# winstonww/ReacherDistilation

Measured on AMD Instinct MI355X. Metric: Reacher env-steps/sec (rollout+distill step) at 1/2/4/8 MI355X; student MSE, higher is better.
Workload: dtype f32; 1 GPU; c4; description=BASELINE config 4: 262,144 envs per GPU, RCCL student-grad all-reduce, MSE, fp32, envs_per_gpu=262144, envs_total=262144, student=MlpPolicy 2x64 tanh (5060 params, f32), teacher=MlpPolicy 2x64 tanh, loss=mse, act_with=teacher, optimizer=TF1 Adam lr 0.0001, 1 step per env-step, parallelism=dp1, collective=none, f32_mode=split

## Files before the change

include/reacher_distill.h:

```cpp
#ifndef REACHER_DISTILL_H
#define REACHER_DISTILL_H
#include <stdint.h>

#include "reacher.h"
#include "reacher_comm.h"

#ifdef __cplusplus
extern "C" {
#endif

#define RDD_LOSS_MSE 0
#define RDD_LOSS_KL 1
#define RDD_ACT_TEACHER 0
#define RDD_ACT_STUDENT 1

typedef struct {
    int64_t n_envs;
    int64_t n_envs_global;
    int64_t env_base;
    uint64_t seed;
    int32_t loss;
    int32_t act_with;
    float lr, beta1, beta2, eps;
    int32_t grid;
    int32_t metrics_len;
    int32_t stagger;
    int32_t student_dtype;
    int32_t accum_steps;
    int32_t f32_split;
    int32_t group_envs;
} rdd_config;

#define RDD_DTYPE_F32 0
#define RDD_DTYPE_BF16 1


#define RDD_STAGGER_GROUP 32

typedef struct rdd_trainer rdd_trainer;

int rdd_create(rdd_trainer** out, const rdd_config* cfg, int device, void* hip_stream);
int rdd_destroy(rdd_trainer* tr);
int rdd_param_count(void);
int rdd_set_stream(rdd_trainer* tr, void* hip_stream);

int rdd_set_teacher(rdd_trainer* tr, const float* params, const float* ob_mean, const float* ob_std);
int rdd_set_student(rdd_trainer* tr, const float* params, const float* ob_mean, const float* ob_std);
int rdd_get_student(rdd_trainer* tr, float* params);

int rdd_reset(rdd_trainer* tr);

int rdd_rollout(rdd_trainer* tr);
int rdd_apply(rdd_trainer* tr);
int rdd_step(rdd_trainer* tr);
int rdd_rollout_accum(rdd_trainer* tr);
int rdd_step_accum(rdd_trainer* tr);
int rdd_rollout_obs(rdd_trainer* tr, const float* obs, int64_t n, int64_t n_global);
int rdd_step_obs(rdd_trainer* tr, const float* obs, int64_t n);
int rdd_rollout_rows(rdd_trainer* tr, const float* obs, const float* t_pdflat, int64_t n, int64_t n_global);
int rdd_step_rows(rdd_trainer* tr, const float* obs, const float* t_pdflat, int64_t n);

#define RDD_STAGE_ROLLOUT 1
#define RDD_STAGE_REDUCE 2
#define RDD_STAGE_APPLY 3
#define RDD_STAGE_REDUCE_APPLY 4
#define RDD_STAGE_REDUCE_ACCUM 5
#define RDD_STAGE_REDUCE_ACCUM_APPLY 6
int rdd_launch_stage(rdd_trainer* tr, int stage);
float* rdd_grad_buffer(rdd_trainer* tr);
int rdd_bind_grad_buffer(rdd_trainer* tr, float* grad);
int rdd_bind_comm(rdd_trainer* tr, rd_comm* comm);
int rdd_allreduce_grad(rdd_trainer* tr);

int rdd_forward(rdd_trainer* tr, const float* obs, int64_t n, float* t_pdflat, float* s_pdflat);

#define RDD_EVAL_TEACHER 0
#define RDD_EVAL_STUDENT 1
typedef struct {
    int64_t n_envs;
    int64_t env_base;
    uint64_t seed;
    int32_t policy;
    int32_t episodes;
    int32_t first_episode;
    int32_t grid;
    const float* draws;
} rdd_eval_config;
int rdd_evaluate(rdd_trainer* tr, const rdd_eval_config* cfg, float* returns, float* final_dist, float* records);

int rdd_get_env_state(rdd_trainer* tr, float* state);
int rdd_set_env_state(rdd_trainer* tr, const float* state);

int rdd_get_counter(rdd_trainer* tr, int64_t* steps);
int rdd_get_counters(rdd_trainer* tr, int64_t* env_steps, int64_t* opt_steps);
int rdd_read_metrics(rdd_trainer* tr, int64_t count, double* out);
int rdd_last_layout(const rdd_trainer* tr, int32_t out[4]);

#ifdef __cplusplus
}
#endif
#endif
```

reacherdistilation_amd/csrc/distill.hip:

```cpp
#include <hip/hip_runtime.h>
#include <stdint.h>

#include <new>

#include "../../include/reacher_distill.h"
#include "rd_comm_impl.h"
#include "rd_common.h"
#include "rd_host.h"
#include "rd_device.h"
#include "rd_physics.h"

namespace {

using rd::f32x4, rd::mfma, rd::ld4, rd::st4, rd::wave_sum, rd::wave_sync, rd::kTanhScale, rd::tanh_pre, rd::load_state;

#ifdef RD_STAMPS
#define STAMP(idx)                                                                      \
    do {                                                                                \
        __builtin_amdgcn_sched_barrier(0);                                              \
        unsigned long long t_;                                                          \
        asm volatile("s_memtime %0\n\ts_waitcnt lgkmcnt(0)" : "=s"(t_)::"memory");     \
        __builtin_amdgcn_sched_barrier(0);                                              \
        if (lane == 0 && a.dbg) a.dbg[(blockIdx.x * WAVES + wave) * NSTAMP + (idx)] += t_;   \
    } while (0)
#define RTSTAMP(idx)                                                                    \
    do {                                                                                \
        __builtin_amdgcn_sched_barrier(0);                                              \
        const unsigned long long t_ = __builtin_amdgcn_s_memrealtime();                 \
        __builtin_amdgcn_sched_barrier(0);                                              \
        if (lane == 0 && a.dbg) a.dbg[(blockIdx.x * WAVES + wave) * NSTAMP + (idx)] += t_;   \
    } while (0)
#else
#define STAMP(idx) do {} while (0)
#define RTSTAMP(idx) do {} while (0)
#endif

#include "distill_layout.h"
#include "distill_forward.h"
#include "distill_reduce.h"
#include "distill_rollout.h"
#include "distill_eval.h"

}

struct rdd_trainer {
    rdd_config cfg{};
    int device = 0;
    hipStream_t stream = nullptr;
    int grid = 0;
    rd::DeviceAllocs mem;
    float* state = nullptr;
    float* tnet = nullptr;
    float* snet = nullptr;
    float* timg = nullptr;
    float* simg = nullptr;
    float* m = nullptr;
    float* v = nullptr;
    float* grad = nullptr;
    float* own_grad = nullptr;
    float* ws = nullptr;
    float* hist = nullptr;
    uint32_t* ctl = nullptr;
    unsigned long long* dbg = nullptr;
    int last_grid = 0;
    int last_gs = GROUP, last_hlp = 0, last_mode = 0;
    int ws_rows = 0;
    int cus = 0;
    int gs = GROUP;
    int accum = 1;
    rd_comm* comm = nullptr;
};

namespace {

int group_envs(int64_t n, int pairs_total, int fixed) {
    if (fixed) return fixed;
    if (n >= (int64_t)GROUP * pairs_total) return 64;
    if (n >= (int64_t)32 * pairs_total) return 32;
    return 16;
}

int teacher_kind(const rdd_trainer* t) { return t->cfg.f32_split ? IMG_SPLIT : IMG_F32; }
int student_kind(const rdd_trainer* t) {
    return t->cfg.student_dtype == RDD_DTYPE_BF16 ? IMG_BF16 : (t->cfg.f32_split ? IMG_SPLIT : IMG_F32);
}
int image_floats(int kind, bool student) {
    if (kind == IMG_SPLIT) return student ? NETX_S : NETX;
    if (kind == IMG_BF16) return NETB_S;
    return student ? NET_S : NET;
}

int grid_for(int64_t n, int gs, int cap) {
    const int64_t want = ((n + gs - 1) / gs + PAIRS - 1) / PAIRS;
    return (int)(want < cap ? want : cap);
}

ReduceArgs reduce_args(const rdd_trainer* t, int reduce, int adam, int accum) {
    ReduceArgs a;
    a.ws = t->ws;
    a.nblk = t->last_grid;
    a.grad = t->grad;
    a.params = t->snet;
    a.m = t->m;
    a.v = t->v;
    a.ctl = t->ctl;
    a.hist = t->hist;
    a.hist_len = t->cfg.metrics_len;
    a.reduce = reduce;
    a.adam = adam;
    a.accum = accum;
    a.bump_env = reduce;
    a.bump_opt = adam;
    a.lr = t->cfg.lr;
    a.b1 = t->cfg.beta1;
    a.b2 = t->cfg.beta2;
    a.eps = t->cfg.eps;
    a.simg = t->simg;
    a.img_kind = student_kind(t);
    a.xerr = rd_comm_device_err(t->comm);
    return a;
}

int launch_rollout(rdd_trainer* t, const float* obs_in = nullptr, int64_t n_obs = 0, int64_t n_obs_global = 0,
                   const float* tflat_in = nullptr, int ksteps = 1) {
    RolloutArgs a;
    a.ksteps = ksteps;
    a.n = obs_in ? n_obs : t->cfg.n_envs;
    a.obs_in = obs_in;
    a.timg = t->timg;
    a.simg = t->simg;
    a.env_base = t->cfg.env_base;
    a.seed = t->cfg.seed;
    a.state = t->state;
    a.tnet = tflat_in ? tflat_in : t->tnet;
    a.snet = t->snet;
    a.ctl = t->ctl;
    a.ws = t->ws;
    a.loss = t->cfg.loss;
    a.act_student = t->cfg.act_with == RDD_ACT_STUDENT;
    a.stagger = t->cfg.stagger;
    a.dbg = t->dbg;
    a.inv_n_global = obs_in ? 1.0f / (float)n_obs_global : 1.0f / ((float)t->cfg.n_envs_global * (float)t->accum);
    int grid = t->grid;
    a.gs = t->gs;
    if (obs_in) {
        a.gs = group_envs(n_obs, t->ws_rows * PAIRS, t->cfg.group_envs);
        grid = grid_for(n_obs, a.gs, t->ws_rows);
    }
    const bool bs = t->cfg.student_dtype == RDD_DTYPE_BF16, spl = t->cfg.f32_split != 0;
    const int64_t ngroups = (a.n + a.gs - 1) / a.gs;
    const bool hlp = !bs && !tflat_in && a.gs == TILE && ngroups <= 2 * (int64_t)t->ws_rows &&
                     t->cfg.group_envs == 0 &&
                     ksteps == 1;
    if (hlp) grid = (int)((ngroups + 1) / 2);
    t->last_grid = grid;
    t->last_gs = a.gs;
    t->last_hlp = hlp;
    t->last_mode = tflat_in ? 2 : (obs_in ? 1 : 0);
    void (*k)(RolloutArgs) =
        bs ? (spl ? rollout_kernel<true, true, true, MD_TEACHER, false, true>
                  : rollout_kernel<true, false, true, MD_TEACHER>)
           : hlp ? (spl ? rollout_kernel<false, true, false, MD_HELPER> : rollout_kernel<false, false, false, MD_HELPER>)
                 : (spl ? rollout_kernel<false, true, false, MD_TEACHER> : rollout_kernel<false, false, false, MD_TEACHER>);
    if (ksteps > 1)
        k = bs ? (spl ? rollout_kernel<true, true, false, MD_TEACHER, true> : rollout_kernel<true, false, false, MD_TEACHER, true>)
               : (spl ? rollout_kernel<false, true, false, MD_TEACHER, true> : rollout_kernel<false, false, false, MD_TEACHER, true>);
    if (tflat_in)
        k = bs ? rollout_kernel<true, false, false, MD_ROWS>
               : (spl ? rollout_kernel<false, true, false, MD_ROWS> : rollout_kernel<false, false, false, MD_ROWS>);
    hipLaunchKernelGGL(k, dim3(grid), dim3(BLOCK), 0, t->stream, a);
    RD_HIP(hipGetLastError(), "rollout_kernel launch");
    return RD_OK;
}

int launch_reduce(rdd_trainer* t, int reduce, int adam, int accum = 0) {
    const ReduceArgs a = reduce_args(t, reduce, adam, accum);
    hipLaunchKernelGGL(reduce_adam_kernel, dim3(RED_GRID), dim3(RED_BLOCK), 0, t->stream, a);
    RD_HIP(hipGetLastError(), "reduce_adam_kernel launch");
    return RD_OK;
}

}

extern "C" {

int rdd_param_count(void) { return P_TOT; }

int rdd_set_stream(rdd_trainer* t, void* hip_stream) {
    if (!t) return rd::set_error(RD_EINVAL, "rdd_set_stream: null handle");
    t->stream = (hipStream_t)hip_stream;
    return RD_OK;
}

int rdd_create(rdd_trainer** out, const rdd_config* cfg, int device, void* hip_stream) {
    if (!out || !cfg) return rd::set_error(RD_EINVAL, "rdd_create: null argument");
    if (cfg->n_envs <= 0 || cfg->n_envs_global < cfg->n_envs || cfg->env_base < 0 ||
        cfg->n_envs > ((int64_t)1 << 31) || (cfg->loss != RDD_LOSS_MSE && cfg->loss != RDD_LOSS_KL) ||
        (cfg->act_with != RDD_ACT_TEACHER && cfg->act_with != RDD_ACT_STUDENT) || !(cfg->lr > 0) ||
        cfg->grid < 0 || cfg->metrics_len < 0 || (cfg->stagger != 0 && cfg->stagger != 1) ||
        (cfg->student_dtype != RDD_DTYPE_F32 && cfg->student_dtype != RDD_DTYPE_BF16) || cfg->accum_steps < 0 ||
        (cfg->f32_split != 0 && cfg->f32_split != 1) ||
        (cfg->group_envs != 0 && cfg->group_envs != 16 && cfg->group_envs != 32 && cfg->group_envs != 64))
        return rd::set_error(RD_EINVAL, "rdd_create: bad config");
    rd::DeviceGuard g(device);
    RD_HIP(g.err, "rdd_create: hipSetDevice");
    rdd_trainer* t = new (std::nothrow) rdd_trainer();
    if (!t) return rd::set_error(RD_EINVAL, "rdd_create: out of host memory");
    t->cfg = *cfg;
    if (t->cfg.metrics_len == 0) t->cfg.metrics_len = 4096;
    t->accum = cfg->accum_steps > 1 ? cfg->accum_steps : 1;
    t->device = device;
    t->stream = (hipStream_t)hip_stream;
    t->cus = rd::cu_count(device);
    const int cap = cfg->grid > 0 ? cfg->grid : t->cus;
    t->ws_rows = cap;
    t->gs = group_envs(cfg->n_envs, cap * PAIRS, cfg->group_envs);
    t->grid = grid_for(cfg->n_envs, t->gs, cap);
    t->last_grid = t->grid;
    t->last_gs = t->gs;
    const size_t netf = P_TOT + 2 * OBD;
    rd::DeviceAllocs& mem = t->mem;
    mem.stream = t->stream;
    mem.zeroed(&t->state, (size_t)8 * cfg->n_envs);
    mem.zeroed(&t->tnet, netf);
    mem.zeroed(&t->snet, netf);
    mem.zeroed(&t->timg, image_floats(teacher_kind(t), false));
    mem.zeroed(&t->simg, image_floats(student_kind(t), true));
    mem.zeroed(&t->m, P_TOT);
    mem.zeroed(&t->v, P_TOT);
    mem.zeroed(&t->own_grad, P_TOT);
    t->grad = t->own_grad;
    mem.zeroed(&t->ws, (size_t)t->ws_rows * P_WS);
    mem.zeroed(&t->hist, (size_t)t->cfg.metrics_len * N_MET);
    mem.zeroed(&t->ctl, 16);
#ifdef RD_STAMPS
    mem.zeroed(&t->dbg, (size_t)t->ws_rows * WAVES * NSTAMP);
#endif
    if (mem.err != hipSuccess) {
        const hipError_t e = mem.err;
        rdd_destroy(t);
        return rd::hip_fail(e, "rdd_create: allocation");
    }
    *out = t;
    return RD_OK;
}

int rdd_destroy(rdd_trainer* t) {
    if (!t) return RD_OK;
    rd::DeviceGuard g(t->device);
    t->mem.free_all();
    delete t;
    return RD_OK;
}

static int set_net(rdd_trainer* t, float* dst, const float* params, const float* mu, const float* sd,
                   const char* what) {
    if (!t || !params || !mu || !sd) return rd::set_error(RD_EINVAL, "%s: null argument", what);
    rd::DeviceGuard g(t->device);
    RD_HIP(g.err, what);
    if (int rc = rd::upload_net(what, dst, params, P_TOT, mu, sd, OBD, t->stream)) return rc;
    const bool student = dst == t->snet;
    const int kind = student ? student_kind(t) : teacher_kind(t);
    hipLaunchKernelGGL(pack_net_kernel, dim3(1), dim3(256), 0, t->stream, dst, student ? t->simg : t->timg,
                       image_floats(kind, student), student ? 1 : 0, kind);
    RD_HIP(hipGetLastError(), what);
    return RD_OK;
}

int rdd_set_teacher(rdd_trainer* t, const float* p, const float* mu, const float* sd) {
    return set_net(t, t ? t->tnet : nullptr, p, mu, sd, "rdd_set_teacher");
}

// ... 223 lines not shown
    RD_HIP(g.err, "rdd_set_env_state");
    const int64_t n = t->cfg.n_envs;
    uint32_t bad = 0;
    RD_HIP(hipMemsetAsync(t->ctl + 14, 0, sizeof(uint32_t), t->stream), "rdd_set_env_state");
    hipLaunchKernelGGL(check_state_kernel, dim3((unsigned)((n + 255) / 256)), dim3(256), 0, t->stream, n, state,
                       t->ctl + 14);
    RD_HIP(hipGetLastError(), "rdd_set_env_state: check_state_kernel launch");
    RD_HIP(hipMemcpyAsync(&bad, t->ctl + 14, sizeof(bad), hipMemcpyDeviceToHost, t->stream), "rdd_set_env_state");
    RD_HIP(hipStreamSynchronize(t->stream), "rdd_set_env_state");
    if (bad)
        return rd::set_error(RD_EINVAL,
                             "rdd_set_env_state: a joint angle outside the fused rollout's range (|q0| < %g, |q1| <= %g "
                             "rad, finite); the gym-API env (rd_set_state) takes any state",
                             (double)rd::kRolloutMaxQ0, (double)rd::kRolloutMaxQ1);
    RD_HIP(hipMemcpyAsync(t->state, state, sizeof(float) * 8 * n, hipMemcpyDeviceToDevice, t->stream),
           "rdd_set_env_state");
    return RD_OK;
}

static int read_ctl(rdd_trainer* t, uint32_t (&c)[16], const char* what) {
    rd::DeviceGuard g(t->device);
    RD_HIP(g.err, what);
    RD_HIP(hipMemcpyAsync(c, t->ctl, sizeof(c), hipMemcpyDeviceToHost, t->stream), what);
    RD_HIP(hipStreamSynchronize(t->stream), what);
    if (c[8]) return rd::set_error(RD_EINVAL, "%s: a rollout's producer/consumer hand-off timed out", what);
    if (c[13]) return rd::set_error(RD_ECOMM, "%s: a gradient exchange failed; its optimiser step was skipped", what);
    return RD_OK;
}

int rdd_get_counter(rdd_trainer* t, int64_t* steps) {
    if (!t || !steps) return rd::set_error(RD_EINVAL, "rdd_get_counter: null argument");
    uint32_t c[16];
    if (int rc = read_ctl(t, c, "rdd_get_counter")) return rc;
    *steps = c[0];
    return RD_OK;
}

int rdd_get_counters(rdd_trainer* t, int64_t* env_steps, int64_t* opt_steps) {
    if (!t) return rd::set_error(RD_EINVAL, "rdd_get_counters: null handle");
    uint32_t c[16];
    if (int rc = read_ctl(t, c, "rdd_get_counters")) return rc;
    if (env_steps) *env_steps = c[0];
    if (opt_steps) *opt_steps = c[1];
    return RD_OK;
}

int rdd_read_metrics(rdd_trainer* t, int64_t count, double* out) {
    if (!t || !out || count < 0) return rd::set_error(RD_EINVAL, "rdd_read_metrics: bad argument");
    int64_t steps = 0;
    if (int rc = rdd_get_counters(t, nullptr, &steps)) return rc;
    return rd::read_ring("rdd_read_metrics", "steps", t->hist, t->cfg.metrics_len, N_MET, steps, count, out);
}

int rdd_last_layout(const rdd_trainer* t, int32_t out[4]) {
    if (!t || !out) return rd::set_error(RD_EINVAL, "rdd_last_layout: null argument");
    out[0] = t->last_gs;
    out[1] = t->last_grid;
    out[2] = t->last_hlp;
    out[3] = t->last_mode;
    return RD_OK;
}

#ifdef RD_STAMPS
int rdd_debug_stamps(rdd_trainer* t, unsigned long long* out, int64_t cap) {
    if (!t || !out || !t->dbg) return rd::set_error(RD_EINVAL, "rdd_debug_stamps: bad argument");
    const int64_t cnt = (int64_t)t->ws_rows * WAVES * NSTAMP;
    if (cap < cnt) return rd::set_error(RD_EINVAL, "rdd_debug_stamps: need %lld", (long long)cnt);
    RD_HIP(hipStreamSynchronize(t->stream), "rdd_debug_stamps");
    RD_HIP(hipMemcpy(out, t->dbg, sizeof(unsigned long long) * cnt, hipMemcpyDeviceToHost), "rdd_debug_stamps");
    RD_HIP(hipMemset(t->dbg, 0, sizeof(unsigned long long) * cnt), "rdd_debug_stamps");
    return (int)cnt;
}
#endif

}
```

reacherdistilation_amd/csrc/distill_rollout.h:

```cpp
#pragma once

struct RolloutArgs {
    int64_t n, env_base;
    uint64_t seed;
    float* state;
    const float* tnet;
    const float* snet;
    uint32_t* ctl;
    float* ws;
    int loss, act_student, stagger;
    float inv_n_global;
    int gs;
    int ksteps;
    unsigned long long* dbg;
    const float* obs_in;
    const float* timg;
    const float* simg;
};

__device__ __forceinline__ bool wait_ge(const uint32_t* f, uint32_t target, uint32_t* err) {
    for (uint32_t spins = 0;; ++spins) {
        if (__hip_atomic_load(f, __ATOMIC_ACQUIRE, __HIP_MEMORY_SCOPE_WORKGROUP) >= target) return true;
        if (spins > SPIN_LIMIT) {
            if ((threadIdx.x & 63) == 0) __hip_atomic_store(err, 1u, __ATOMIC_RELAXED, __HIP_MEMORY_SCOPE_AGENT);
            return false;
        }
        __builtin_amdgcn_s_sleep(1);
    }
}

__device__ __forceinline__ void publish(uint32_t* f, uint32_t v) {
    __hip_atomic_store(f, v, __ATOMIC_RELEASE, __HIP_MEMORY_SCOPE_WORKGROUP);
}

__device__ __forceinline__ float env_step_group(const RolloutArgs& a, uint32_t C, int64_t i, bool valid, float act0,
                                                float act1, rd::State& st, float& met_n) {
    const uint32_t iu = (uint32_t)i;
    const float rew = rd::env_step<false>(st, act0, act1);
    const int64_t gid = a.env_base + i;
    const uint32_t u = C + (a.stagger ? (uint32_t)((gid / RDD_STAGGER_GROUP) % rd::kEpisodeSteps) : 0u);
    const bool done_step = (u % rd::kEpisodeSteps) == rd::kEpisodeSteps - 1;
    if (done_step) {
        float dr[6];
        rd::philox_draw(a.seed, (uint64_t)gid, u / rd::kEpisodeSteps + 1, dr);
        rd::env_reset(st, dr);
    }
    if (!valid) return 0.0f;
    rd::store_state(a.state, a.n, iu, st, done_step);
    met_n += 1.0f;
    return rew;
}

constexpr int MD_TEACHER = 0, MD_ROWS = 1, MD_HELPER = 2;
template <bool BS, bool SPL, bool CP, int MD, bool KS = false, bool TC = false>
__global__ __launch_bounds__(BLOCK, 2) void rollout_kernel(RolloutArgs a) {
    constexpr bool TGT = MD == MD_ROWS, HLP = MD == MD_HELPER;
    static_assert(!TC || (BS && MD == MD_TEACHER && !KS), "teacher on the consumer: bf16 student, K = 1");
    constexpr int P_TM = CP ? P_ACT : P_SACT;
    static_assert(!HLP || !BS, "helper pairs: f32 student kernels only");
    constexpr int TN = TGT ? 0 : img_t(SPL), SN = img_s(BS, SPL);
    __shared__ __attribute__((aligned(16))) float lds[TN + SN + PAIRS * PSCR];
    float* LT = lds;
    float* LS = lds + TN;
    const int wave = threadIdx.x >> 6, lane = threadIdx.x & 63;
    const int j = lane & 15, g = lane >> 4;
    const int pair = wave & (PAIRS - 1);
    const bool producer = wave < PAIRS;
    uint32_t* flags = reinterpret_cast<uint32_t*>(lds + TN + SN + pair * PSCR + P_FLAGS);
    uint32_t* err = a.ctl + 8;

    RTSTAMP(16);
    STAMP(0);
    const int gs = a.gs;
    const uint32_t n32 = (uint32_t)a.n;
    const uint32_t ngroups = (n32 + (uint32_t)gs - 1) / (uint32_t)gs;
    static_assert(!KS || (!CP && MD == MD_TEACHER), "K-step launches: teacher mode, producer-side env step");
    if constexpr (KS) {
        if (a.obs_in) {
            if (threadIdx.x == 0) __hip_atomic_store(a.ctl + 8, 1u, __ATOMIC_RELAXED, __HIP_MEMORY_SCOPE_AGENT);
            return;
        }
    }
    if constexpr (HLP) {
        if (ngroups > 2u * gridDim.x) {
            if (threadIdx.x == 0) __hip_atomic_store(a.ctl + 8, 1u, __ATOMIC_RELAXED, __HIP_MEMORY_SCOPE_AGENT);
            return;
        }
    }
    const bool helper = HLP && pair >= 2;
    const uint32_t gstride = gridDim.x * (HLP ? 2 : PAIRS);
    const uint32_t gfirst = helper ? ngroups : blockIdx.x * (HLP ? 2 : PAIRS) + pair;
    rd::State st0{};
    if (producer && !a.obs_in && gfirst < ngroups && lane < gs && gfirst * gs + lane < a.n)
        load_state(a.state, a.n, (uint32_t)(gfirst * gs + lane), st0);
    const uint32_t og = blockIdx.x * 2 + (pair & 1);
    const bool hstep = helper && producer && !a.obs_in && !a.act_student;
    if constexpr (HLP) {
        if (hstep && og < ngroups && lane < gs && og * gs + lane < a.n)
            load_state(a.state, a.n, (uint32_t)(og * gs + lane), st0);
    }
    static_assert(NET % 4 == 0 && NET_S % 4 == 0, "16-B images");
    float* PS = lds + TN + SN + pair * PSCR;
    const bool first_obs = producer && gfirst < ngroups;
    auto group_obs = [&](uint32_t k, uint32_t i, bool lvalid, rd::State& st) {
        float ob[OBD];
        if (a.obs_in) {
#pragma unroll
            for (int q = 0; q < OBD; ++q) ob[q] = lvalid ? a.obs_in[(size_t)i * OBD + q] : 0.0f;
        } else {
            rd::observe<false>(st, ob);
// ... 64 lines not shown
            STAMP(8);
            const uint32_t Ck = C + kk;
            const uint32_t base = grp * (uint32_t)gs;
            const uint32_t i = base + (uint32_t)lane;
            const bool lvalid = lane < gs && i < n32;
            float* obs = PS + P_SO;
            float* act = PS + P_ACT;
            rd::State st{};
            if (k == 0) {
                st = st0;
            } else if (resident) {
                if (lvalid) st = st0;
                group_obs(k, i, lvalid, st);
            } else {
                if (!a.obs_in && lvalid) load_state(a.state, a.n, i, st);
                group_obs(k, i, lvalid, st);
            }
            STAMP(11);
            wave_sync();
            if constexpr (TC) publish(flags + 2, k + 1);
            const int ntile = (int)min((uint32_t)(gs / TILE), (n32 - base + TILE - 1) / TILE);
            for (int t = 0; t < ntile; ++t) {
                const bool tvalid = base + TILE * t + j < a.n;
                const float* obt = obs + TILE * t * SOS;
                f32x4 H1[4], H2[4];
                float mt0, mt1, ms0, ms1;
                float rl0 = tl0, rl1 = tl1, rr0 = rtv0, rr1 = rtv1;
                STAMP(10);
                if constexpr (TGT) {
                    const uint32_t row = base + TILE * t + j;
                    const f32x4 tq = tvalid ? ld4(a.tnet + (size_t)row * 4) : f32x4{0.f, 0.f, 0.f, 0.f};
                    if constexpr (BS) mlp_forward_bf16(LS, obt, j, g, H1, H2, ms0, ms1);
                    else if constexpr (SPL) mlp_forward_split_t<true>(LS, obt, j, g, H1, H2, ms0, ms1);
                    else mlp_forward(LS, obt, j, g, H1, H2, ms0, ms1);
                    mt0 = tq[0];
                    mt1 = tq[1];
                    rl0 = tq[2];
                    rl1 = tq[3];
                    rr0 = 1.0f / __expf(2.0f * rl0);
                    rr1 = 1.0f / __expf(2.0f * rl1);
                } else if constexpr (HLP) {
                    if (k == 0) {
                        if constexpr (SPL) mlp_forward_split_t<true>(LS, obt, j, g, H1, H2, ms0, ms1);
                        else mlp_forward<true>(LS, obt, j, g, H1, H2, ms0, ms1);
                        const float* hp = lds + TN + SN + (pair + 2) * PSCR;
                        if (!(ok = wait_ge(reinterpret_cast<const uint32_t*>(hp + P_FLAGS), 1u, err))) break;
                        mt0 = hp[P_ACT + 2 * j];
                        mt1 = hp[P_ACT + 2 * j + 1];
                    } else {
                        if constexpr (SPL) mlp_forward_pair_split(LT, LS, obt, j, g, H1, H2, mt0, mt1, ms0, ms1);
                        else mlp_forward_pair<true>(LT, LS, obt, j, g, H1, H2, mt0, mt1, ms0, ms1);
                    }
                } else if constexpr (BS) {
                    if (TC && (t & 1)) {
                        mlp_forward_bf16(LS, obt, j, g, H1, H2, ms0, ms1);
                        if (!(ok = wait_ge(flags + 3, ++tct, err))) break;
                        mt0 = PS[P_TM + 2 * j];
                        mt1 = PS[P_TM + 2 * j + 1];
                    } else {
                    if constexpr (SPL) mlp_forward_split(LT, obt, j, g, mt0, mt1);
                    else mlp_forward<CP || KS || TC>(LT, obt, j, g, H1, H2, mt0, mt1);
                    mlp_forward_bf16(LS, obt, j, g, H1, H2, ms0, ms1);
                    }
                } else {
                    if constexpr (SPL) mlp_forward_pair_split(LT, LS, obt, j, g, H1, H2, mt0, mt1, ms0, ms1);
                    else mlp_forward_pair<false, kPairFence>(LT, LS, obt, j, g, H1, H2, mt0, mt1, ms0, ms1);
                }
                STAMP(12);
                const float d0 = ms0 - mt0, d1 = ms1 - mt1;
                float dm0, dm1, dl0 = 0.0f, dl1 = 0.0f, lossv;
                if (a.loss == RDD_LOSS_MSE) {
                    dm0 = d0 * a.inv_n_global;
                    dm1 = d1 * a.inv_n_global;
                    lossv = (d0 * d0 + d1 * d1) * (0.5f * a.inv_n_global);
                } else {
                    dm0 = d0 * rr0;
                    dm1 = d1 * rr1;
                    dl0 = sv0 * rr0 - 1.0f;
                    dl1 = sv1 * rr1 - 1.0f;
                    lossv = (rl0 - sl0 + (sv0 + d0 * d0) * (0.5f * rr0) - 0.5f) +
                            (rl1 - sl1 + (sv1 + d1 * d1) * (0.5f * rr1) - 0.5f);
                }
                if (!tvalid) { dm0 = dm1 = dl0 = dl1 = 0.0f; }
                if (g == 0 && tvalid) {
                    met_l += lossv;
                    met_m += d0 * d0 + d1 * d1;
                    gb3a += dm0; gb3b += dm1; gls0 += dl0; gls1 += dl1;
                    if (!CP) {
                        act[(TILE * t + j) * 2] = a.act_student ? ms0 : mt0;
                        act[(TILE * t + j) * 2 + 1] = a.act_student ? ms1 : mt1;
                    }
                }
                f32x4 dZ[4];
#pragma unroll
                for (int fb = 0; fb < 4; ++fb) {
                    const f32x4 wa = ld4(LS + SW3 + (16 * fb + 4 * g) * 2);
                    const f32x4 wb = ld4(LS + SW3 + (16 * fb + 4 * g) * 2 + 4);
                    const float w0[4] = {wa[0], wa[2], wb[0], wb[2]}, w1[4] = {wa[1], wa[3], wb[1], wb[3]};
#pragma unroll
                    for (int r = 0; r < 4; ++r) {
                        const float h = H2[fb][r];
                        gw3a[fb][r] = fmaf(h, dm0, gw3a[fb][r]);
                        gw3b[fb][r] = fmaf(h, dm1, gw3b[fb][r]);
                        dZ[fb][r] = fmaf(w0[r], dm0, w1[r] * dm1) * fmaf(-h, h, 1.0f);
                    }
                }
                STAMP(2);
                if (!(ok = wait_ge(flags + 1, tiles, err))) break;
                STAMP(3);
                float* h1t = PS + P_H1T;
                float* dzt = PS + P_DZT;
#pragma unroll
                for (int fb = 0; fb < 4; ++fb) {
                    st4(h1t + j * SAS + 16 * fb + 4 * g, H1[fb]);
                    st4(dzt + j * SAS + 16 * fb + 4 * g, dZ[fb]);
                }
                if (lane < TILE * SOS / 4) st4(PS + P_SOB + 4 * lane, ld4(obt + 4 * lane));
                if (CP && g == 0) {
                    PS[P_SACT + 2 * j] = a.act_student ? ms0 : mt0;
// ... 269 lines not shown
                const float* OP = lds + TN + SN + (pair & 1) * PSCR;
                STAMP(20);
                ok = wait_ge(reinterpret_cast<const uint32_t*>(OP + P_FLAGS), 1u, err);
                STAMP(21);
                if (ok) {
                    const float* h1t = OP + P_H1T;
                    const float* dzt = OP + P_DZT;
                    if constexpr (SPL) {
                        float x32[2][8], y32[2][8];
#pragma unroll
                        for (int e = 0; e < 8; ++e)
#pragma unroll
                            for (int b = 0; b < 2; ++b) {
                                x32[b][e] = h1t[(8 * h32 + e) * SAS + 32 * b + c32];
                                y32[b][e] = dzt[(8 * h32 + e) * SAS + 32 * b + c32];
                            }
#pragma unroll
                        for (int b = 0; b < 2; ++b)
                            gb2s[b] += ((y32[b][0] + y32[b][1]) + (y32[b][2] + y32[b][3])) +
                                       ((y32[b][4] + y32[b][5]) + (y32[b][6] + y32[b][7]));
                        dw2_split32(x32, y32, gW2s);
                    } else {
                    float x[4][4], y[4][4];
#pragma unroll
                    for (int s = 0; s < 4; ++s)
#pragma unroll
                        for (int b = 0; b < 4; ++b) {
                            x[s][b] = h1t[(4 * s + g) * SAS + 16 * b + j];
                            y[s][b] = dzt[(4 * s + g) * SAS + 16 * b + j];
                        }
#pragma unroll
                        for (int s = 0; s < 4; ++s) {
#pragma unroll
                            for (int b = 0; b < 4; ++b) gb2[b] += y[s][b];
#pragma unroll
                            for (int mb = 0; mb < 4; ++mb) {
                                fence_begin<true>(gW2[mb]);
#pragma unroll
                                for (int nb = 0; nb < 4; ++nb) gW2[mb][nb] = mfma(x[s][mb], y[s][nb], gW2[mb][nb]);
                                fence_end<true>(gW2[mb]);
                            }
                        }
                    }
                }
                STAMP(22);
            }
        }
        uint32_t gi = 0, tcc = 0;
        for (uint32_t kk = 0;; ++kk) {
        for (uint32_t grp = gfirst; ok && grp < ngroups; grp += gstride, ++gi) {
            const uint32_t base = grp * (uint32_t)gs;
            const int ntile = (int)min((uint32_t)(gs / TILE), (n32 - base + TILE - 1) / TILE);
            if constexpr (TC) {
                if (!(ok = wait_ge(flags + 2, gi + 1, err))) break;
            }
            for (int t = 0; ok && t < ntile; ++t) {
                if constexpr (TC) {
                    if (!(t & 1) && t + 1 < ntile) {
                        const float* obt = PS + P_SO + TILE * (t + 1) * SOS;
                        float m0, m1;
                        if constexpr (SPL) {
                            mlp_forward_split(LT, obt, j, g, m0, m1);
                        } else {
                            f32x4 h1[4], h2[4];
                            mlp_forward<true>(LT, obt, j, g, h1, h2, m0, m1);
                        }
                        if (g == 0) {
                            PS[P_TM + 2 * j] = m0;
                            PS[P_TM + 2 * j + 1] = m1;
                        }
                        publish(flags + 3, ++tcc);
                    }
                }
                ok = bwd_tile(t);
            }
            if (!ok) break;
            end_group(base, C + kk);
        }
        if (!KS || !ok || kk + 1 >= (uint32_t)a.ksteps) break;
        }
#pragma unroll
        for (int x = 0; x < 4; ++x) gb2[x] = xsum32(xsum16(gb2[x]));
#pragma unroll
        for (int x = 0; x < 2; ++x) gb2s[x] = xsum32(gb2s[x]);
        if constexpr (CP) { met_r = wave_sum(met_r); met_n = wave_sum(met_n); }
        STAMP(6);
        __syncthreads();
        STAMP(9);
        float* R = lds + pair * RPAD;
        if constexpr (D32) {
#pragma unroll
            for (int mb = 0; mb < 2; ++mb)
#pragma unroll
                for (int nb = 0; nb < 2; ++nb)
#pragma unroll
                    for (int r = 0; r < 16; ++r)
                        R[(12 + 32 * mb + (r & 3) + 8 * (r >> 2) + 4 * h32) * RROW + 32 * nb + c32] = gW2s[mb][nb][r];
        } else {
#pragma unroll
        for (int mb = 0; mb < 4; ++mb)
#pragma unroll
            for (int nb = 0; nb < 4; ++nb)
#pragma unroll
                for (int r = 0; r < 4; ++r) R[(12 + 16 * mb + 4 * g + r) * RROW + 16 * nb + j] = gW2[mb][nb][r];
        }
        if (g < 3) {
#pragma unroll
            for (int nb = 0; nb < 4; ++nb)
#pragma unroll
                for (int r = 0; r < 4; ++r) R[(4 * g + r) * RROW + 16 * nb + j] = gW1[nb][r];
        }
        if constexpr (D32) {
            if (h32 == 0) {
#pragma unroll
                for (int nb = 0; nb < 2; ++nb) R[RSHIFT + P_B2 + 32 * nb + c32] = gb2s[nb];
            }
        } else if (g == 0) {
#pragma unroll
// ... 23 lines not shown
```

reacherdistilation_amd/distill.py:

```python
from __future__ import annotations

import ctypes
from dataclasses import dataclass

import numpy as np
import torch

from . import _native as nat
from .dist import allreduce_sum_, replicas_identical, shard
from .policy import P_TOT, MlpPolicyParams, student_init, synthetic_teacher

P = nat.P
I32, I64, U64, F32, INT = nat.I32, nat.I64, nat.U64, nat.F32, nat.INT

LOSSES = {"mse": 0, "kl": 1}
ACTORS = {"teacher": 0, "student": 1}
DTYPES = {"f32": 0, "bf16": 1}


class RddConfig(ctypes.Structure):
    _fields_ = [("n_envs", I64), ("n_envs_global", I64), ("env_base", I64), ("seed", U64),
                ("loss", I32), ("act_with", I32), ("lr", F32), ("beta1", F32), ("beta2", F32),
                ("eps", F32), ("grid", I32), ("metrics_len", I32), ("stagger", I32),
                ("student_dtype", I32), ("accum_steps", I32), ("f32_split", I32), ("group_envs", I32)]


class RddEvalConfig(ctypes.Structure):
    _fields_ = [("n_envs", I64), ("env_base", I64), ("seed", U64), ("policy", I32), ("episodes", I32),
                ("first_episode", I32), ("grid", I32), ("draws", P)]


@dataclass
class EvalResult:
    returns: torch.Tensor
    final_dist: torch.Tensor | None = None
    records: torch.Tensor | None = None
    state: torch.Tensor | None = None


nat.register({
    "rdd_evaluate": (INT, [P, ctypes.POINTER(RddEvalConfig), P, P, P]),
    "rdd_create": (INT, [ctypes.POINTER(P), ctypes.POINTER(RddConfig), INT, P]),
    "rdd_destroy": (INT, [P]),
    "rdd_param_count": (INT, []),
    "rdd_set_stream": (INT, [P, P]),
    "rdd_set_teacher": (INT, [P, P, P, P]),
    "rdd_set_student": (INT, [P, P, P, P]),
    "rdd_get_student": (INT, [P, P]),
    "rdd_reset": (INT, [P]),
    "rdd_rollout": (INT, [P]),
    "rdd_apply": (INT, [P]),
    "rdd_step": (INT, [P]),
    "rdd_rollout_accum": (INT, [P]),
    "rdd_step_accum": (INT, [P]),
    "rdd_launch_stage": (INT, [P, INT]),
    "rdd_grad_buffer": (P, [P]),
    "rdd_bind_grad_buffer": (INT, [P, P]),
    "rdd_forward": (INT, [P, P, I64, P, P]),
    "rdd_get_env_state": (INT, [P, P]),
    "rdd_set_env_state": (INT, [P, P]),
    "rdd_get_counter": (INT, [P, ctypes.POINTER(I64)]),
    "rdd_get_counters": (INT, [P, ctypes.POINTER(I64), ctypes.POINTER(I64)]),
    "rdd_rollout_obs": (INT, [P, P, I64, I64]),
    "rdd_step_obs": (INT, [P, P, I64]),
    "rdd_rollout_rows": (INT, [P, P, P, I64, I64]),
    "rdd_step_rows": (INT, [P, P, P, I64]),
    "rdd_read_metrics": (INT, [P, I64, P]),
    "rdd_last_layout": (INT, [P, ctypes.POINTER(I32)]),
    "rdd_bind_comm": (INT, [P, P]),
    "rdd_allreduce_grad": (INT, [P]),
})


@dataclass
class DistillConfig:
    n_envs: int = 4096
    n_envs_global: int = 0
    seed: int = 0
    loss: str = "mse"
    act_with: str = "teacher"
    lr: float = 1e-4
    beta1: float = 0.9
    beta2: float = 0.999
    eps: float = 1e-8
    teacher_seed: int = 1
    student_seed: int = 2
    grid: int = 0
    metrics_len: int = 4096
    stagger: bool = True
    student_dtype: str = "f32"
    accum_steps: int = 1
    f32_split: bool = True
    group_envs: int = 0


class DistillTrainer:
    def __init__(self, cfg: DistillConfig, device="cuda:0", rank: int = 0, world_size: int = 1,
                 process_group=None, teacher: MlpPolicyParams | None = None,
                 student: MlpPolicyParams | None = None, comm=None):
        self.cfg = cfg
        self.device = torch.device(device)
        if self.device.type != "cuda":
            raise ValueError("DistillTrainer runs on a GPU (HIP) device only; there is no CPU path")
        if self.device.index is None:
            self.device = torch.device("cuda", torch.cuda.current_device())
        self.rank, self.world = rank, world_size
        self.pg = process_group
        self._lib = nat.load()
        assert self._lib.rdd_param_count() == P_TOT
        if cfg.n_envs_global > 0:
            self.n_local, self.env_base = shard(cfg.n_envs_global, rank, world_size)
            self.n_global = cfg.n_envs_global
        else:
            self.n_local, self.env_base = cfg.n_envs, cfg.n_envs * rank
            self.n_global = cfg.n_envs * world_size
        c = RddConfig(n_envs=self.n_local, n_envs_global=self.n_global, env_base=self.env_base,
                      seed=cfg.seed % 2 ** 64, loss=LOSSES[cfg.loss], act_with=ACTORS[cfg.act_with], lr=cfg.lr,
                      beta1=cfg.beta1, beta2=cfg.beta2, eps=cfg.eps, grid=cfg.grid, metrics_len=cfg.metrics_len,
                      stagger=int(bool(cfg.stagger)), student_dtype=DTYPES[cfg.student_dtype],
                      accum_steps=max(1, int(cfg.accum_steps)), f32_split=int(bool(cfg.f32_split)),
                      group_envs=int(cfg.group_envs))
        h = ctypes.c_void_p()
        with torch.cuda.device(self.device):
            nat.check(self._lib.rdd_create(ctypes.byref(h), ctypes.byref(c), self.device.index or 0,
                                           nat.stream_handle(self.device)), "rdd_create")
        self._h = h
        self.teacher = teacher or synthetic_teacher(cfg.teacher_seed)
        self.student = student or student_init(cfg.student_seed)
        self.set_teacher(self.teacher)
        self.set_student(self.student)
        self.reset()
        self._grad = torch.zeros(P_TOT, dtype=torch.float32, device=self.device)
        nat.check(self._lib.rdd_bind_grad_buffer(self._h, nat.ptr(self._grad)), "rdd_bind_grad_buffer")
        self.steps = 0
        self._k = 0
        self.comm = None
        if comm is not None:
            self.bind_comm(comm)

    def bind_comm(self, comm):
        if comm is not None:
            if comm.world != self.world or comm.rank != self.rank:
                raise ValueError(f"communicator rank {comm.rank} of {comm.world} for a trainer at rank "
                                 f"{self.rank} of {self.world}")
            if comm.device != self.device:
                raise ValueError(f"communicator on {comm.device} for a trainer on {self.device}")
        nat.check(self._lib.rdd_bind_comm(self._h, comm.handle if comm is not None else None), "rdd_bind_comm")
        self.comm = comm

    def set_teacher(self, p: MlpPolicyParams):
        f, mu, sd = p.device_tensors(self.device)
        nat.check(self._lib.rdd_set_teacher(self._h, nat.ptr(f), nat.ptr(mu), nat.ptr(sd)), "rdd_set_teacher")
        torch.cuda.current_stream(self.device).synchronize()

    def set_student(self, p: MlpPolicyParams):
        f, mu, sd = p.device_tensors(self.device)
        nat.check(self._lib.rdd_set_student(self._h, nat.ptr(f), nat.ptr(mu), nat.ptr(sd)), "rdd_set_student")
        torch.cuda.current_stream(self.device).synchronize()

    def student_params(self) -> torch.Tensor:
        out = torch.empty(P_TOT, dtype=torch.float32, device=self.device)
        nat.check(self._lib.rdd_get_student(self._h, nat.ptr(out)), "rdd_get_student")
        return out

    def reset(self):
        nat.check(self._lib.rdd_reset(self._h), "rdd_reset")
        self.steps = 0

    def step(self):
        K = max(1, int(self.cfg.accum_steps))
        if K == 1:
            if self.world == 1 or self.comm is not None:
                nat.check(self._lib.rdd_step(self._h), "rdd_step")
            else:
# ... 34 lines not shown
        obs = self._obs_arg(obs)
        n = obs.shape[0]
        if self.world == 1:
            nat.check(self._lib.rdd_step_obs(self._h, nat.ptr(obs), n), "rdd_step_obs")
        else:
            nat.check(self._lib.rdd_rollout_obs(self._h, nat.ptr(obs), n, n * self.world), "rdd_rollout_obs")
            self.allreduce_grad()
            nat.check(self._lib.rdd_apply(self._h), "rdd_apply")
        self._keep = obs
        self.steps += 1

    def rollout_obs(self, obs: torch.Tensor, n_global: int | None = None):
        obs = self._obs_arg(obs)
        nat.check(self._lib.rdd_rollout_obs(self._h, nat.ptr(obs), obs.shape[0], n_global or obs.shape[0]),
                  "rdd_rollout_obs")
        self._keep = obs

    def step_rows(self, obs: torch.Tensor, t_pdflat: torch.Tensor):
        obs, tp = self._obs_arg(obs), self._tflat_arg(t_pdflat, obs.shape[0])
        n = obs.shape[0]
        if self.world == 1:
            nat.check(self._lib.rdd_step_rows(self._h, nat.ptr(obs), nat.ptr(tp), n), "rdd_step_rows")
        else:
            nat.check(self._lib.rdd_rollout_rows(self._h, nat.ptr(obs), nat.ptr(tp), n, n * self.world),
                      "rdd_rollout_rows")
            self.allreduce_grad()
            nat.check(self._lib.rdd_apply(self._h), "rdd_apply")
        self._keep = (obs, tp)
        self.steps += 1

    def rollout_rows(self, obs: torch.Tensor, t_pdflat: torch.Tensor, n_global: int | None = None):
        obs, tp = self._obs_arg(obs), self._tflat_arg(t_pdflat, obs.shape[0])
        nat.check(self._lib.rdd_rollout_rows(self._h, nat.ptr(obs), nat.ptr(tp), obs.shape[0],
                                             n_global or obs.shape[0]), "rdd_rollout_rows")
        self._keep = (obs, tp)

    def _tflat_arg(self, t, n):
        t = torch.as_tensor(t).to(self.device, torch.float32).contiguous()
        if t.dim() != 2 or t.shape != (n, 4):
            raise ValueError("t_pdflat must be [n, 4] (teacher mean | logstd per row)")
        return t

    def _obs_arg(self, obs):
        obs = torch.as_tensor(obs).to(self.device, torch.float32).contiguous()
        if obs.dim() != 2 or obs.shape[1] != 11 or obs.shape[0] == 0:
            raise ValueError("obs must be [n, 11]")
        return obs

    def counters(self):
        e, o = ctypes.c_int64(), ctypes.c_int64()
        nat.check(self._lib.rdd_get_counters(self._h, ctypes.byref(e), ctypes.byref(o)), "rdd_get_counters")
        return e.value, o.value

    def last_layout(self):
        out = (I32 * 4)()
        nat.check(self._lib.rdd_last_layout(self._h, out), "rdd_last_layout")
        return out[0], out[1], bool(out[2]), ("env", "obs", "rows")[out[3]]

    def set_stream(self, stream: torch.cuda.Stream):
        nat.check(self._lib.rdd_set_stream(self._h, ctypes.c_void_p(stream.cuda_stream)), "rdd_set_stream")

    def capture(self, steps: int = 1, fused: bool = False) -> torch.cuda.CUDAGraph:
        if self.world != 1:
            raise RuntimeError("graph capture is for the single-rank step")
        g = torch.cuda.CUDAGraph()
        prev = torch.cuda.current_stream(self.device)
        torch.cuda.synchronize(self.device)
        if not fused and max(1, int(self.cfg.accum_steps)) > 1 and steps % self.cfg.accum_steps:
            raise ValueError("capture whole optimiser steps: steps must be a multiple of accum_steps")
        s0 = self.steps
        with torch.cuda.graph(g):
            self.set_stream(torch.cuda.current_stream(self.device))
            for _ in range(steps):
                self.step_accum() if fused else self.step()
        self.steps = s0
        self.set_stream(prev)
        return g

    STAGE_ROLLOUT, STAGE_REDUCE, STAGE_APPLY, STAGE_REDUCE_APPLY = 1, 2, 3, 4
    STAGE_REDUCE_ACCUM, STAGE_REDUCE_ACCUM_APPLY = 5, 6

    def launch(self, stage: int):
        nat.check(self._lib.rdd_launch_stage(self._h, stage), "rdd_launch_stage")

    def rollout(self):
        nat.check(self._lib.rdd_rollout(self._h), "rdd_rollout")

    def apply(self):
        nat.check(self._lib.rdd_apply(self._h), "rdd_apply")
        self.steps += 1

    def grad(self) -> torch.Tensor:
        return self._grad

    def allreduce_grad(self):
        if self.comm is not None:
            nat.check(self._lib.rdd_allreduce_grad(self._h), "rdd_allreduce_grad")
        else:
            allreduce_sum_(self._grad, self.pg)

    def replicas_identical(self) -> bool:
        return replicas_identical(self.student_params(), self.pg)

    def forward(self, obs: torch.Tensor, teacher=True, student=True):
        obs = obs.to(self.device, torch.float32).contiguous()
        n = obs.shape[0]
        t = torch.empty(n, 4, device=self.device) if teacher else None
        s = torch.empty(n, 4, device=self.device) if student else None
        nat.check(self._lib.rdd_forward(self._h, nat.ptr(obs), n, nat.ptr(t) if t is not None else None,
                                        nat.ptr(s) if s is not None else None), "rdd_forward")
# ... 60 lines not shown
```

Measured before the change: 3.427 billion env-steps/s.

## Offload teacher forward for selected tiles to consumer waves in f32 split kernel

```diff
diff --git a/include/reacher_distill.h b/include/reacher_distill.h
--- a/include/reacher_distill.h
+++ b/include/reacher_distill.h
@@ -29,6 +29,7 @@
     int32_t accum_steps;
     int32_t f32_split;
     int32_t group_envs;
+    int32_t teacher_tiles;
 } rdd_config;
 
 #define RDD_DTYPE_F32 0
@@ -94,7 +95,7 @@
 int rdd_get_counter(rdd_trainer* tr, int64_t* steps);
 int rdd_get_counters(rdd_trainer* tr, int64_t* env_steps, int64_t* opt_steps);
 int rdd_read_metrics(rdd_trainer* tr, int64_t count, double* out);
-int rdd_last_layout(const rdd_trainer* tr, int32_t out[4]);
+int rdd_last_layout(const rdd_trainer* tr, int32_t out[5]);
 
 #ifdef __cplusplus
 }
diff --git a/reacherdistilation_amd/csrc/distill.hip b/reacherdistilation_amd/csrc/distill.hip
--- a/reacherdistilation_amd/csrc/distill.hip
+++ b/reacherdistilation_amd/csrc/distill.hip
@@ -64,6 +64,8 @@
     unsigned long long* dbg = nullptr;
     int last_grid = 0;
     int last_gs = GROUP, last_hlp = 0, last_mode = 0;
+    int last_tcm = 0;
+    int tcm = 0;
     int ws_rows = 0;
     int cus = 0;
     int gs = GROUP;
@@ -94,6 +96,9 @@
     const int64_t want = ((n + gs - 1) / gs + PAIRS - 1) / PAIRS;
     return (int)(want < cap ? want : cap);
 }
+
+constexpr int kTeacherTilesDefault = 0b0010;
+bool teacher_tiles_ok(int m) { return m == -1 || m == 0 || m == 0b0010 || m == 0b1010 || m == 0b1110; }
 
 ReduceArgs reduce_args(const rdd_trainer* t, int reduce, int adam, int accum) {
     ReduceArgs a;
@@ -157,11 +162,17 @@
     t->last_gs = a.gs;
     t->last_hlp = hlp;
     t->last_mode = tflat_in ? 2 : (obs_in ? 1 : 0);
+    const int tcm = !bs && spl && !hlp && !tflat_in && ksteps == 1 ? t->tcm : 0;
+    t->last_tcm = bs && spl && !tflat_in && ksteps == 1 ? 0b1010 : tcm;
     void (*k)(RolloutArgs) =
-        bs ? (spl ? rollout_kernel<true, true, true, MD_TEACHER, false, true>
+        bs ? (spl ? rollout_kernel<true, true, true, MD_TEACHER, false, 0b1010>
                   : rollout_kernel<true, false, true, MD_TEACHER>)
            : hlp ? (spl ? rollout_kernel<false, true, false, MD_HELPER> : rollout_kernel<false, false, false, MD_HELPER>)
-                 : (spl ? rollout_kernel<false, true, false, MD_TEACHER> : rollout_kernel<false, false, false, MD_TEACHER>);
+                 : (spl ? (tcm == 0b1110   ? rollout_kernel<false, true, false, MD_TEACHER, false, 0b1110>
+                           : tcm == 0b1010 ? rollout_kernel<false, true, false, MD_TEACHER, false, 0b1010>
+                           : tcm == 0b0010 ? rollout_kernel<false, true, false, MD_TEACHER, false, 0b0010>
+                                           : rollout_kernel<false, true, false, MD_TEACHER>)
+                        : rollout_kernel<false, false, false, MD_TEACHER>);
     if (ksteps > 1)
         k = bs ? (spl ? rollout_kernel<true, true, false, MD_TEACHER, true> : rollout_kernel<true, false, false, MD_TEACHER, true>)
                : (spl ? rollout_kernel<false, true, false, MD_TEACHER, true> : rollout_kernel<false, false, false, MD_TEACHER, true>);
@@ -202,6 +213,9 @@
         (cfg->f32_split != 0 && cfg->f32_split != 1) ||
         (cfg->group_envs != 0 && cfg->group_envs != 16 && cfg->group_envs != 32 && cfg->group_envs != 64))
         return rd::set_error(RD_EINVAL, "rdd_create: bad config");
+    if (!teacher_tiles_ok(cfg->teacher_tiles))
+        return rd::set_error(RD_EINVAL, "rdd_create: teacher_tiles %d is not built (-1 default, 0, 2 = 0b0010, "
+                                        "10 = 0b1010, 14 = 0b1110)", (int)cfg->teacher_tiles);
     rd::DeviceGuard g(device);
     RD_HIP(g.err, "rdd_create: hipSetDevice");
     rdd_trainer* t = new (std::nothrow) rdd_trainer();
@@ -218,6 +232,7 @@
     t->grid = grid_for(cfg->n_envs, t->gs, cap);
     t->last_grid = t->grid;
     t->last_gs = t->gs;
+    t->tcm = cfg->teacher_tiles < 0 ? kTeacherTilesDefault : cfg->teacher_tiles;
     const size_t netf = P_TOT + 2 * OBD;
     rd::DeviceAllocs& mem = t->mem;
     mem.stream = t->stream;
@@ -547,12 +562,13 @@
     return rd::read_ring("rdd_read_metrics", "steps", t->hist, t->cfg.metrics_len, N_MET, steps, count, out);
 }
 
-int rdd_last_layout(const rdd_trainer* t, int32_t out[4]) {
+int rdd_last_layout(const rdd_trainer* t, int32_t out[5]) {
     if (!t || !out) return rd::set_error(RD_EINVAL, "rdd_last_layout: null argument");
     out[0] = t->last_gs;
     out[1] = t->last_grid;
     out[2] = t->last_hlp;
     out[3] = t->last_mode;
+    out[4] = t->last_tcm;
     return RD_OK;
 }
 
diff --git a/reacherdistilation_amd/csrc/distill_rollout.h b/reacherdistilation_amd/csrc/distill_rollout.h
--- a/reacherdistilation_amd/csrc/distill_rollout.h
+++ b/reacherdistilation_amd/csrc/distill_rollout.h
@@ -29,6 +29,18 @@
     }
 }
 
+__device__ __forceinline__ bool wait_ge_uniform(const uint32_t* f, uint32_t target, uint32_t* err) {
+    for (uint32_t spins = 0;; ++spins) {
+        const uint32_t v = __hip_atomic_load(f, __ATOMIC_ACQUIRE, __HIP_MEMORY_SCOPE_WORKGROUP);
+        if (__builtin_amdgcn_readfirstlane(v) >= target) return true;
+        if (spins > SPIN_LIMIT) {
+            if ((threadIdx.x & 63) == 0) __hip_atomic_store(err, 1u, __ATOMIC_RELAXED, __HIP_MEMORY_SCOPE_AGENT);
+            return false;
+        }
+        __builtin_amdgcn_s_sleep(1);
+    }
+}
+
 __device__ __forceinline__ void publish(uint32_t* f, uint32_t v) {
     __hip_atomic_store(f, v, __ATOMIC_RELEASE, __HIP_MEMORY_SCOPE_WORKGROUP);
 }
@@ -52,10 +64,14 @@
 }
 
 constexpr int MD_TEACHER = 0, MD_ROWS = 1, MD_HELPER = 2;
-template <bool BS, bool SPL, bool CP, int MD, bool KS = false, bool TC = false>
+template <bool BS, bool SPL, bool CP, int MD, bool KS = false, int TCM = 0>
 __global__ __launch_bounds__(BLOCK, 2) void rollout_kernel(RolloutArgs a) {
     constexpr bool TGT = MD == MD_ROWS, HLP = MD == MD_HELPER;
-    static_assert(!TC || (BS && MD == MD_TEACHER && !KS), "teacher on the consumer: bf16 student, K = 1");
+    constexpr bool TC = TCM != 0;
+    static_assert(TCM == 0 || (MD == MD_TEACHER && !KS && SPL), "teacher on the consumer: split teacher, K = 1");
+    static_assert((TCM & ~((1 << GROUP / TILE) - 2)) == 0, "a mask over tiles 1 .. 3; tile 0 stays on the producer");
+    auto tc_tile = [](int t) { return TCM == 0b1010 ? (t & 1) != 0 : ((TCM >> t) & 1) != 0; };
+    auto tc_next = [](int t) { return TCM == 0b1010 ? !(t & 1) : ((TCM >> (t + 1)) & 1) != 0; };
     constexpr int P_TM = CP ? P_ACT : P_SACT;
     static_assert(!HLP || !BS, "helper pairs: f32 student kernels only");
     constexpr int TN = TGT ? 0 : img_t(SPL), SN = img_s(BS, SPL);
@@ -226,7 +242,7 @@
                         else mlp_forward_pair<true>(LT, LS, obt, j, g, H1, H2, mt0, mt1, ms0, ms1);
                     }
                 } else if constexpr (BS) {
-                    if (TC && (t & 1)) {
+                    if (TC && tc_tile(t)) {
                         mlp_forward_bf16(LS, obt, j, g, H1, H2, ms0, ms1);
                         if (!(ok = wait_ge(flags + 3, ++tct, err))) break;
                         mt0 = PS[P_TM + 2 * j];
@@ -237,8 +253,18 @@
                     mlp_forward_bf16(LS, obt, j, g, H1, H2, ms0, ms1);
                     }
                 } else {
-                    if constexpr (SPL) mlp_forward_pair_split(LT, LS, obt, j, g, H1, H2, mt0, mt1, ms0, ms1);
-                    else mlp_forward_pair<false, kPairFence>(LT, LS, obt, j, g, H1, H2, mt0, mt1, ms0, ms1);
+                    if constexpr (SPL) {
+                        if (TC && tc_tile(t)) {
+                            mlp_forward_split_t<true>(LS, obt, j, g, H1, H2, ms0, ms1);
+                            if (!(ok = wait_ge_uniform(flags + 3, ++tct, err))) break;
+                            mt0 = PS[P_TM + 2 * j];
+                            mt1 = PS[P_TM + 2 * j + 1];
+                        } else {
+                            mlp_forward_pair_split(LT, LS, obt, j, g, H1, H2, mt0, mt1, ms0, ms1);
+                        }
+                    } else {
+                        mlp_forward_pair<false, kPairFence>(LT, LS, obt, j, g, H1, H2, mt0, mt1, ms0, ms1);
+                    }
                 }
                 STAMP(12);
                 const float d0 = ms0 - mt0, d1 = ms1 - mt1;
@@ -614,18 +640,18 @@
             const uint32_t base = grp * (uint32_t)gs;
             const int ntile = (int)min((uint32_t)(gs / TILE), (n32 - base + TILE - 1) / TILE);
             if constexpr (TC) {
-                if (!(ok = wait_ge(flags + 2, gi + 1, err))) break;
+                if (!(ok = BS ? wait_ge(flags + 2, gi + 1, err) : wait_ge_uniform(flags + 2, gi + 1, err))) break;
             }
             for (int t = 0; ok && t < ntile; ++t) {
                 if constexpr (TC) {
-                    if (!(t & 1) && t + 1 < ntile) {
+                    if (tc_next(t) && t + 1 < ntile) {
                         const float* obt = PS + P_SO + TILE * (t + 1) * SOS;
                         float m0, m1;
-                        if constexpr (SPL) {
-                            mlp_forward_split(LT, obt, j, g, m0, m1);
-                        } else {
-                            f32x4 h1[4], h2[4];
-                            mlp_forward<true>(LT, obt, j, g, h1, h2, m0, m1);
+                        STAMP(18);
+                        mlp_forward_split(LT, obt, j, g, m0, m1);
+                        STAMP(19);
+                        if constexpr ((TCM & (TCM >> 1)) != 0) {
+                            if (tc_tile(t) && !(ok = wait_ge_uniform(flags, tiles + 1, err))) break;
                         }
                         if (g == 0) {
                             PS[P_TM + 2 * j] = m0;
diff --git a/reacherdistilation_amd/distill.py b/reacherdistilation_amd/distill.py
--- a/reacherdistilation_amd/distill.py
+++ b/reacherdistilation_amd/distill.py
@@ -22,7 +22,8 @@
     _fields_ = [("n_envs", I64), ("n_envs_global", I64), ("env_base", I64), ("seed", U64),
                 ("loss", I32), ("act_with", I32), ("lr", F32), ("beta1", F32), ("beta2", F32),
                 ("eps", F32), ("grid", I32), ("metrics_len", I32), ("stagger", I32),
-                ("student_dtype", I32), ("accum_steps", I32), ("f32_split", I32), ("group_envs", I32)]
+                ("student_dtype", I32), ("accum_steps", I32), ("f32_split", I32), ("group_envs", I32),
+                ("teacher_tiles", I32)]
 
 
 class RddEvalConfig(ctypes.Structure):
@@ -92,6 +93,7 @@
     accum_steps: int = 1
     f32_split: bool = True
     group_envs: int = 0
+    teacher_tiles: int = -1
 
 
 class DistillTrainer:
@@ -119,7 +121,7 @@
                       beta1=cfg.beta1, beta2=cfg.beta2, eps=cfg.eps, grid=cfg.grid, metrics_len=cfg.metrics_len,
                       stagger=int(bool(cfg.stagger)), student_dtype=DTYPES[cfg.student_dtype],
                       accum_steps=max(1, int(cfg.accum_steps)), f32_split=int(bool(cfg.f32_split)),
-                      group_envs=int(cfg.group_envs))
+                      group_envs=int(cfg.group_envs), teacher_tiles=int(cfg.teacher_tiles))
         h = ctypes.c_void_p()
         with torch.cuda.device(self.device):
             nat.check(self._lib.rdd_create(ctypes.byref(h), ctypes.byref(c), self.device.index or 0,
@@ -260,10 +262,11 @@
         nat.check(self._lib.rdd_get_counters(self._h, ctypes.byref(e), ctypes.byref(o)), "rdd_get_counters")
         return e.value, o.value
 
-    def last_layout(self):
-        out = (I32 * 4)()
+    def last_layout(self, teacher_tiles: bool = False):
+        out = (I32 * 5)()
         nat.check(self._lib.rdd_last_layout(self._h, out), "rdd_last_layout")
-        return out[0], out[1], bool(out[2]), ("env", "obs", "rows")[out[3]]
+        lay = out[0], out[1], bool(out[2]), ("env", "obs", "rows")[out[3]]
+        return lay + (out[4],) if teacher_tiles else lay
 
     def set_stream(self, stream: torch.cuda.Stream):
         nat.check(self._lib.rdd_set_stream(self._h, ctypes.c_void_p(stream.cuda_stream)), "rdd_set_stream")
```

After: 3.482 billion env-steps/s (median of 6 runs). 1.02x the previous value.
